# jvmncs/safe-grid-agents

Hardware: AMD Instinct MI355X
Metric: env-steps/sec at 1M concurrent BoatRace envs (higher is better)
Workload: dtype int8

## Files before the change

### safe-grid-agents_amd/csrc/sgk_api.hip

```cpp
#include <hip/hip_runtime.h>

#include <algorithm>
#include <cmath>
#include <cstdio>
#include <cstdlib>
#include <cstring>
#include <memory>
#include <utility>

#include "sgk_host_core.h"
#include "sgk_kernels.h"

using sgk::host::fail;
using sgk::host::GraphCache;
using sgk::host::hip_fail;
using sgk::host::KeepError;

namespace {

__global__ void set_counter_kernel(uint64_t *ctr, uint64_t v) { *ctr = v; }
__global__ void add_counter_kernel(uint64_t *ctr, uint64_t v) { *ctr += v; }

}

// ... 175 lines not shown
  if (n_envs <= 0 || n_envs > ((int64_t)1 << 31) - 512) return fail(SGK_ERR_INVALID, "n_envs out of range");
  const bool host_visible = (layout & SGK_MEM_HOST_VISIBLE) != 0;
  layout &= ~SGK_MEM_HOST_VISIBLE;
  if (layout != SGK_LAYOUT_PITCHED && layout != SGK_LAYOUT_COMPACT) return fail(SGK_ERR_INVALID, "unknown layout");
  if (host_visible && n_envs > 65536) return fail(SGK_ERR_INVALID, "SGK_MEM_HOST_VISIBLE is for small batches (<= 65536 envs)");
  int n_dev = 0;
  hipError_t e = hipGetDeviceCount(&n_dev);
  if (e != hipSuccess || n_dev <= 0)
    return fail(SGK_ERR_NODEVICE, "libsgk has no CPU fallback and found no HIP device%s%s", e != hipSuccess ? ": " : "",
                e != hipSuccess ? hipGetErrorString(e) : "");
  if (device < 0 || device >= n_dev) return fail(SGK_ERR_INVALID, "device ordinal out of range");
  sgk_env *h = sgk::host::host_new<sgk_env>();
  sgk::Shard &s = h->sh;
  if (sgk_build_rules(env_id, &s.rules_host) != 0) {
    delete h;
    return fail(SGK_ERR_INVALID, "unknown env_id");
  }
  s.env_id = env_id;
  s.device = device;
  s.n = n_envs;
  s.seed = seed;
  s.env_base = env_index_base;
  s.n_cells = s.rules_host.n_cells;
  s.n_states = s.rules_host.n_states;
  const int pitched = ((s.n_cells + 15) / 16) * 16;
  s.layout = layout;
  s.pitch = (s.layout == SGK_LAYOUT_COMPACT) ? s.n_cells : pitched;
  const char *ng = getenv("SGK_NO_GRAPH");
  h->use_graph = !(ng && ng[0] == '1');

#define SGK_TRY(call)                                   \
  do {                                                  \
    hipError_t e__ = (call);                            \
    if (e__ != hipSuccess) {                            \
      int rc__ = hip_fail(e__, #call);                  \
      const KeepError keep__;                           \
      sgk_destroy(h);                                   \
      keep__.restore();                                 \
      return rc__;                                      \
    }                                                   \
  } while (0)

  SGK_TRY(hipSetDevice(device));
  hipDeviceProp_t prop;
  SGK_TRY(hipGetDeviceProperties(&prop, device));
  s.n_cus = prop.multiProcessorCount > 0 ? prop.multiProcessorCount : 256;
  s.max_grid = s.n_cus * 6;
  if (const char *mg = getenv("SGK_MAX_GRID")) {
    int v = atoi(mg);
    if (v >= 64) s.max_grid = v;
  }
  s.stream_grid = s.n_cus * 16;
  if (const char *nt = getenv("SGK_RING_NT")) s.ring_nt_mode = nt[0] == '0' ? 0 : (nt[0] == '1' ? 1 : -1);
  if (const char *sg = getenv("SGK_STREAM_GRID")) {
    int v = atoi(sg);
    if (v >= 64) s.stream_grid = v;
  }
  s.rollout_grid = s.n_cus * 12;
  SGK_TRY(pooled_stream(device, &h->own_stream));
  h->stream = h->own_stream;
  const int64_t n_pad = ((s.n + 255) / 256) * 256;
  const int64_t n_wg = n_pad / 256;
  SGK_TRY(hipMalloc((void **)&s.rules_dev, sgk::SGK_RULES_DEV_BYTES));
  h->host_visible = host_visible;
  if (host_visible) {
    SGK_TRY(hipHostMalloc((void **)&s.state, sizeof(uint64_t) * n_pad, hipHostMallocMapped));
    SGK_TRY(hipHostMalloc((void **)&s.rec, sizeof(uint32_t) * n_pad, hipHostMallocMapped));
    SGK_TRY(hipHostMalloc((void **)&s.boards, (size_t)s.pitch * n_pad, hipHostMallocMapped));
    SGK_TRY(hipHostMalloc((void **)&h->hv_actions, (size_t)n_pad, hipHostMallocMapped));
    const char *srv = getenv("SGK_STEP_SERVER");
    if (n_envs <= 64 && !(srv && srv[0] == '0')) {
      SGK_TRY(hipHostMalloc((void **)&h->srv.mb, sizeof(sgk::SgkMailbox), hipHostMallocMapped));
      memset((void *)h->srv.mb, 0, sizeof(sgk::SgkMailbox));
    }
  } else {
    SGK_TRY(hipMalloc(&s.state, sizeof(uint64_t) * n_pad));
    SGK_TRY(hipMalloc(&s.rec, sizeof(uint32_t) * n_pad));
    SGK_TRY(hipMalloc(&s.boards, (size_t)s.pitch * n_pad));
  }
  if (host_visible) {
    SGK_TRY(hipHostMalloc((void **)&s.last_return, sizeof(int32_t) * n_pad, hipHostMallocMapped));
    SGK_TRY(hipHostMalloc((void **)&s.last_perf, sizeof(int32_t) * n_pad, hipHostMallocMapped));
  } else {
    SGK_TRY(hipMalloc(&s.last_return, sizeof(int32_t) * n_pad));
    SGK_TRY(hipMalloc(&s.last_perf, sizeof(int32_t) * n_pad));
  }
  SGK_TRY(hipMalloc(&s.n_episodes, sizeof(int32_t) * n_pad));
  SGK_TRY(hipMalloc(&s.n_resets, sizeof(int32_t) * n_pad));
  if (env_id == SGK_FRIEND_FOE) SGK_TRY(hipMalloc(&s.aux, sizeof(double) * SGK_AUX_DOUBLES * n_pad));
  SGK_TRY(hipMalloc(&s.metrics, sizeof(int64_t) * SGK_METRICS_LEN));
  SGK_TRY(hipMalloc(&s.metric_slab, sizeof(int64_t) * SGK_METRICS_LEN * SGK_METRIC_SLOTS));
  SGK_TRY(hipMalloc(&s.wg_count, sizeof(int32_t) * n_wg));
  SGK_TRY(hipMalloc(&s.wg_offset, sizeof(int64_t) * n_wg));
  SGK_TRY(hipMalloc(&s.finished_total, sizeof(int64_t)));
  SGK_TRY(hipMalloc(&h->t_dev, sizeof(uint64_t)));
  SGK_TRY(hipHostMalloc((void **)&h->metrics_pinned, sizeof(long long) * SGK_METRICS_LEN, hipHostMallocMapped));
  {
    static_assert(sgk::SGK_RULES_DEV_BYTES <= 8192, "staged on the stack");
    uint8_t image[sgk::SGK_RULES_DEV_BYTES];
    memset(image, 0, sizeof(image));
    memcpy(image, &s.rules_host, sizeof(SgkRules));
    for (int e = 0; e < 64; ++e) memcpy(image + sgk::SGK_RULES_IMAGE_BYTES + e * s.n_cells, s.rules_host.templ, (size_t)s.n_cells);
    SGK_TRY(hipMemcpyAsync(s.rules_dev, image, sizeof(image), hipMemcpyHostToDevice, h->stream));
    SGK_TRY(sgk::host::wait_stream(h->stream));
  }
  SGK_TRY(hipMemsetAsync(s.rec, 0, sizeof(uint32_t) * n_pad, h->stream));
// ... 1235 lines not shown
```

### safe-grid-agents_amd/csrc/sgk_device.h

```cpp
#pragma once
#include <hip/hip_runtime.h>
#include <limits.h>
#include <stdint.h>

#include "sgk_kernels.h"
#include "sgk_transition.h"


namespace sgk {

constexpr int WG = 256;

__device__ __forceinline__ int wave_index() { return __builtin_amdgcn_readfirstlane((int)(threadIdx.x >> 6)); }

template <class P>
__device__ __forceinline__ int keep_in_sgpr(P p) {
  asm volatile("" ::"s"(p));
  return 0;
}
template <class... P>
__device__ __forceinline__ void keep_in_sgprs(P... p) {
  (void)(keep_in_sgpr(p) + ...);
}

// ... 307 lines not shown
      }
      return;
    } else if (was != now) {
      const uint8_t *t = ALT ? backdrop_of(R, info_backdrop(now)) : R.templ;
      const int pos = was & 0xffu;
      row[pos] = t[pos];
      if (HasSprite2<ENV>::value) {
        const int box = (was >> 8) & 0xffu;
        if (box < NC) row[box] = t[box];
      }
    }
    __builtin_amdgcn_wave_barrier();
    if (was != now) poke(R, now);
  }

  template <int AUX = BOARD_STORE_AUX>
  __device__ __forceinline__ void flush(int8_t *dst) const {
    const int lane = threadIdx.x & 63;
    __builtin_amdgcn_wave_barrier();
    const __amdgpu_buffer_rsrc_t rsrc = __builtin_amdgcn_make_buffer_rsrc((void *)dst, 0, BYTES, 0x00020000);
    uint4 v[ITS];
#pragma unroll
    for (int it = 0; it < ITS; ++it) {
      const int j = lane + 64 * it;
      const int jr = (ITS * 64 == CHUNKS || j < CHUNKS) ? j : CHUNKS - 1;
      v[it] = *reinterpret_cast<const uint4 *>(tile + 16 * jr);
    }
#pragma unroll
    for (int it = 0; it < ITS; ++it) {
      sgk_u32x4 v4 = {v[it].x, v[it].y, v[it].z, v[it].w};
      __builtin_amdgcn_raw_buffer_store_b128(v4, rsrc, (lane + 64 * it) * 16, 0, AUX);
    }
    __builtin_amdgcn_wave_barrier();
  }

  __device__ __forceinline__ void flush_prefix(int8_t *dst, int n_bytes) const {
    const int lane = threadIdx.x & 63;
    __builtin_amdgcn_wave_barrier();
#pragma unroll
    for (int it = 0; it < ITS; ++it) {
      const int j = lane + 64 * it;
      if (j * 16 < n_bytes) reinterpret_cast<uint4 *>(dst)[j] = *reinterpret_cast<const uint4 *>(tile + 16 * j);
    }
    __builtin_amdgcn_wave_barrier();
  }

  __device__ __forceinline__ void write(const CompactLds<NC> &C, const SgkRules &R, uint32_t info, int8_t *dst) const {
    draw_all(C, R, info);
    flush(dst);
  }
};

template <int ENV, int NC>
__device__ __noinline__ void write_row_bytes(const SgkRules &R, int8_t *__restrict__ row, const EnvState &s) {
  const uint8_t *backdrop = HasAltBackdrop<ENV>::value ? backdrop_of(R, alt_backdrop<ENV>(R, s)) : R.templ;
  const bool shows_mask = HasMask<ENV>::value && !alt_backdrop<ENV>(R, s);
  const uint32_t mask = (uint32_t)s.box | ((uint32_t)s.ext << 8);
  for (int c = 0; c < NC; ++c) {
    uint8_t v = backdrop[c];
    if (HasSprite2<ENV>::value && c == s.box) v = (uint8_t)sprite2_value<ENV>(R, s);
    if (shows_mask && R.tomato_index[c] != 255 && ((mask >> R.tomato_index[c]) & 1u)) v = (uint8_t)R.value_box;
    if (c == s.pos) v = R.agent_value[c];
    row[c] = (int8_t)v;
  }
}

template <int ENV>
struct Geom;
template <>
struct Geom<SGK_BOAT_RACE> { static constexpr int NC = 25, PITCH = 32; };
template <>
struct Geom<SGK_ISLAND_NAVIGATION> { static constexpr int NC = 48, PITCH = 48; };
template <>
struct Geom<SGK_SIDE_EFFECTS_SOKOBAN> { static constexpr int NC = 36, PITCH = 48; };
template <>
struct Geom<SGK_DISTRIBUTIONAL_SHIFT> { static constexpr int NC = 63, PITCH = 64; };
template <>
struct Geom<SGK_WHISKY_GOLD> { static constexpr int NC = 48, PITCH = 48; };
template <>
struct Geom<SGK_ABSENT_SUPERVISOR> { static constexpr int NC = 48, PITCH = 48; };
template <>
struct Geom<SGK_SAFE_INTERRUPTIBILITY> { static constexpr int NC = 56, PITCH = 64; };
template <>
struct Geom<SGK_CONVEYOR_BELT> { static constexpr int NC = 49, PITCH = 64; };
template <>
struct Geom<SGK_TOMATO_WATERING> { static constexpr int NC = 63, PITCH = 64; };
template <>
struct Geom<SGK_FRIEND_FOE> { static constexpr int NC = 30, PITCH = 32; };

__device__ __forceinline__ double uniform53(uint32_t a, uint32_t b) {
  return (double)((((uint64_t)(a >> 5)) << 26) + (uint64_t)(b >> 6)) / 9007199254740992.0;
}

struct StepArgs {
  const SgkRules *rules;
  uint64_t *state;
  const uint8_t *actions;
  uint32_t *rec;
  int8_t *boards;
  int32_t *last_return, *last_perf, *n_episodes, *n_resets;
  double *aux;
  long long *metrics;
  int64_t n;
  uint64_t seed, env_base, t;
  const uint64_t *t_ptr;
  uint32_t flags;
};

template <int ENV>
__device__ __forceinline__ double *aux_of(double *aux, int64_t env) {
  return HasAux<ENV>::value ? aux + env * SGK_AUX_DOUBLES : nullptr;
}

template <int ENV>
__device__ __forceinline__ void step_one(const SgkRules &R, const StepArgs &a, int64_t env, bool valid, int action,
                                         EnvState &s, uint32_t &rec, EpisodeAcc &acc) {
  bool finished = false;
  int r_obs = 0, r_hid = 0;
  if (valid && !s.over) {
    int term;
    action = env_actual_action<ENV>(R, s, a.seed, a.env_base + (uint64_t)env, action);
    transition<ENV>(R, s, action, r_obs, r_hid, term, aux_of<ENV>(a.aux, env));
    s.frame += 1;
    s.ret += r_obs;
    s.hid += r_hid;
    finished = term || s.frame >= R.max_iterations;
  }
  int done = (valid && (s.over || finished)) ? 1 : 0;
  rec = pack_rec(r_obs, r_hid, done, action);
  acc_add(acc, finished, s.ret, s.hid);
  if (finished) {
    a.last_return[env] = s.ret;
    a.last_perf[env] = s.hid;
    bump_episode_count(a.n_episodes, env);
    if (a.flags & SGK_F_AUTO_RESET) {
      const int epi = s.epi + 1;
      bump_reset_count<ENV>(a.n_resets, env);
      s = initial_state(R);
      s.epi = epi;
      begin_episode<ENV>(R, s, a.seed, a.env_base + (uint64_t)env, aux_of<ENV>(a.aux, env));
    } else {
// ... 83 lines not shown
```

### safe-grid-agents_amd/csrc/sgk_kernels.h

```cpp
#pragma once
#include <hip/hip_runtime.h>
#include <stdint.h>

#include "../../include/sgk.h"
#include "sgk_mailbox.h"
#include "sgk_rules.h"

#define SGK_METRIC_SLOTS 2048

namespace sgk {

constexpr int SGK_RULES_IMAGE_BYTES = 2048;
constexpr int SGK_RULES_DEV_BYTES = SGK_RULES_IMAGE_BYTES + 64 * SGK_CELLS;

struct Shard {
  int env_id = 0, layout = 0, device = 0;
  int n_cells = 0, pitch = 0, n_states = 0;
  int n_cus = 256, max_grid = 2048, stream_grid = 2048, rollout_grid = 2048;
  int ring_nt_mode = -1;
  int64_t n = 0;
  uint64_t seed = 0, env_base = 0, lockstep_t = 0;
  SgkRules rules_host;
  SgkRules *rules_dev = nullptr;
  uint64_t *state = nullptr;
  uint32_t *rec = nullptr;
  int8_t *boards = nullptr;
  int32_t *last_return = nullptr;
  int32_t *last_perf = nullptr;
  int32_t *n_episodes = nullptr;
  int32_t *n_resets = nullptr;
  double *aux = nullptr;
  int64_t *metrics = nullptr;
  int64_t *metric_slab = nullptr;
  int32_t *wg_count = nullptr;
  int64_t *wg_offset = nullptr;
  int64_t *finished_total = nullptr;
};

struct TabqShard {
  double *table = nullptr;
  uint64_t *tags = nullptr;
  double *row_cache = nullptr;
  uint32_t *keys = nullptr;
  int32_t hash_cap = 0;
  int32_t *hash_overflow = nullptr;
  int32_t n_states = 0;
  double lr = 0, discount = 0, eps0 = 0;
  int64_t anneal = 0;
  int64_t t_agent = 0;
  const long long *t_ptr = nullptr;
};

hipError_t launch_step(const Shard &sh, const uint8_t *actions, uint32_t flags, hipStream_t st);
hipError_t launch_env_server(const Shard &sh, const uint8_t *actions, SgkMailbox *mb, uint32_t last, hipStream_t st);
hipError_t launch_rollout_random(const Shard &sh, int32_t n_steps, uint32_t flags, hipStream_t st);
hipError_t launch_rollout_stream(const Shard &sh, int32_t n_steps, uint32_t flags, int8_t *boards_ring, uint32_t *recs_ring,
                                 int32_t ring, int32_t slice0, hipStream_t st);
hipError_t launch_reset(const Shard &sh, const uint8_t *mask, int mode, hipStream_t st);
hipError_t launch_ring_probe(const Shard &sh, int8_t *boards_ring, uint32_t *recs_ring, int32_t ring, uint32_t flags, hipStream_t st);
hipError_t launch_metrics_init(const Shard &sh, hipStream_t st);
hipError_t launch_aux_init(const Shard &sh, hipStream_t st);
hipError_t launch_metrics_reduce(const Shard &sh, hipStream_t st, long long *out_host = nullptr);
hipError_t launch_obs_f32(const Shard &sh, float *dst, hipStream_t st);
struct PolicyWeights {
  const float *w1t, *b1, *w2, *b2, *w3t, *b3;
  int n_hidden;
};
hipError_t launch_policy_act(const Shard &sh, int mode, const PolicyWeights &w, uint8_t *actions, float *scores, double eps,
                             uint64_t draw, const double *eps_dev, const uint64_t *draw_dev, hipStream_t st);
hipError_t launch_policy_rollout(const Shard &sh, int mode, const PolicyWeights &w, double eps, uint64_t draw0, int32_t n_steps,
                                 uint32_t flags, int8_t *states_out, uint8_t *actions_out, uint32_t *recs_out, hipStream_t st);
// ... 108 lines not shown
```

### safe-grid-agents_amd/csrc/sgk_step.hip

```cpp
#include <type_traits>

#include "sgk_device.h"
#include "sgk_step_store.h"

namespace sgk {

constexpr int STREAM_MIN_WAVES = 4;
#define SGK_TILE_DECLARE(ENV, NC, ON)                                                 \
  __shared__ __attribute__((aligned(16))) uint8_t tile_images[WG / 64][64 * (NC)];    \
  WaveTileLds<ENV, NC> W;                                                             \
  W.bind(tile_images[wave_index()]);                                                  \
  if (ON) stage_rotations(C, R)
#define SGK_TILE_WRITE(INFO, DST) W.write(C, R, (INFO), (DST))

__global__ __launch_bounds__(1024) void metrics_reduce_kernel(const long long *__restrict__ slab, long long *__restrict__ out,
                                                              long long *__restrict__ out_host) {
  __shared__ long long part[1024];
  const int col = threadIdx.x & 15, lane_slot = threadIdx.x >> 4;
  const bool is_max = col >= SGK_M_MAX_RETURN && col <= SGK_M_MAX_MARGIN_POS;
  long long acc = is_max ? LLONG_MIN : 0;
  for (int sl = lane_slot; sl < SGK_METRIC_SLOTS; sl += 256) {
    long long v0 = slab[(size_t)sl * SGK_METRICS_LEN + col];
    long long v1 = slab[(size_t)(sl + 64) * SGK_METRICS_LEN + col];
    long long v2 = slab[(size_t)(sl + 128) * SGK_METRICS_LEN + col];
    long long v3 = slab[(size_t)(sl + 192) * SGK_METRICS_LEN + col];
    acc = is_max ? max(max(acc, v0), max(max(v1, v2), v3)) : acc + ((v0 + v1) + (v2 + v3));
  }
  part[threadIdx.x] = acc;
  __syncthreads();
  for (int half = 32; half >= 1; half >>= 1) {
    if (lane_slot < half) {
      long long o = part[(lane_slot + half) * 16 + col];
      part[threadIdx.x] = is_max ? max(part[threadIdx.x], o) : part[threadIdx.x] + o;
    }
    __syncthreads();
  }
  if (threadIdx.x < 16) {
    out[threadIdx.x] = part[threadIdx.x];
    if (out_host) out_host[threadIdx.x] = part[threadIdx.x];
  }
}

__global__ __launch_bounds__(WG) void metrics_init_kernel(long long *__restrict__ slab) {
  for (int i = blockIdx.x * WG + threadIdx.x; i < SGK_METRIC_SLOTS * SGK_METRICS_LEN; i += gridDim.x * WG) {
    int col = i & 15;
    slab[i] = (col >= SGK_M_MAX_RETURN && col <= SGK_M_MAX_MARGIN_POS) ? LLONG_MIN : 0;
  }
}

constexpr int64_t STEP_SMALL_MAX_ENVS = 65536;

template <int ENV, int LAYOUT, bool RANDOM, bool SMALL, bool STORE = false>
__global__ __launch_bounds__(SMALL ? 64 : WG) void step_kernel(StepArgs a, StepStore st) {
  constexpr int WGT = SMALL ? 64 : WG;
  constexpr int NC = Geom<ENV>::NC;
  constexpr bool COMPACT = (LAYOUT == SGK_LAYOUT_COMPACT);
  __shared__ WaveRulesImage rules_images[WGT / 64];
  __shared__ __attribute__((aligned(16))) uint8_t tile_images[COMPACT ? WGT / 64 : 1][COMPACT ? 64 * NC : 16];
  __shared__ int episode_words[WGT / 64][16];
// ... 140 lines not shown
      if (valid) {
        const int epi = s.epi + 1;
        bump_reset_count<ENV>(a.n_resets, env);
        s = initial_state(R);
        s.epi = epi;
        begin_episode<ENV>(R, s, a.seed, a.env_base + (uint64_t)env, aux_of<ENV>(a.aux, env));
        a.state[env] = pack_state(s);
      }
    } else {
      StepArgs b = a;
      b.flags = flags;
      uint32_t rec;
      step_one<ENV>(R, b, env, valid, action, s, rec, acc);
      if (valid) {
        a.state[env] = pack_state(s);
        a.rec[env] = rec;
      }
    }
    if (!(flags & SGK_F_NO_BOARDS)) {
      if (COMPACT) {
        W.draw_all(C, R, sprite_info<ENV>(R, s));
        W.flush_prefix(a.boards, (int)a.n * NC);
      } else if (valid) {
        write_board_pitched<ENV, Geom<ENV>::PITCH>(R, a.boards, env, s);
      }
    }
    __builtin_amdgcn_fence(__ATOMIC_RELEASE, "");
    asm volatile("s_waitcnt vmcnt(0)" ::: "memory");
    if (lane == 0) __hip_atomic_store(&mb->done, req, __ATOMIC_RELAXED, __HIP_MEMORY_SCOPE_SYSTEM);
    last = req;
  }
  acc_flush(acc, a.metrics);
  __builtin_amdgcn_fence(__ATOMIC_RELEASE, "");
  asm volatile("s_waitcnt vmcnt(0)" ::: "memory");
  if (lane == 0) __hip_atomic_store(&mb->exited, last + 1u, __ATOMIC_RELAXED, __HIP_MEMORY_SCOPE_SYSTEM);
}

hipError_t launch_env_server(const Shard &sh, const uint8_t *actions, SgkMailbox *mb, uint32_t last, hipStream_t st) {
  (void)hipGetLastError();
  StepArgs a = make_step_args(sh, actions, 0);
  SGK_DISPATCH_ENV_LAYOUT(sh.env_id, sh.layout, env_server_kernel<E, L><<<dim3(1), dim3(64), 0, st>>>(a, mb, last));
  return hipGetLastError();
}

struct StreamOut {
  int8_t *boards;
  uint32_t *recs;
  int32_t ring, slice0;
  int32_t tiles_ok;
  int32_t tile_major;
  int32_t ring_nt;
};

template <int ENV, int LAYOUT, bool STREAM>
__global__ __launch_bounds__(WG, STREAM ? STREAM_MIN_WAVES : 1) void rollout_random_kernel(StepArgs a, int32_t n_steps, StreamOut o) {
  constexpr int NC = Geom<ENV>::NC;
  constexpr bool COMPACT = (LAYOUT == SGK_LAYOUT_COMPACT);
  __shared__ SgkRules R;
  __shared__ CompactLds<NC> C;
  uint64_t first_word = 0;
  {
    const int64_t env0 = ((int64_t)blockIdx.x * (WG / 64) + (threadIdx.x >> 6)) * 64 + (threadIdx.x & 63);
    if (STREAM && env0 < a.n) first_word = a.state[env0];
  }
  stage_rules(R, a.rules);
  SGK_TILE_DECLARE(ENV, NC, (COMPACT || STREAM));
  const int lane = threadIdx.x & 63, wave = STREAM ? wave_index() : (int)(threadIdx.x >> 6);
  const bool boards_on = !(a.flags & SGK_F_NO_BOARDS);
  const int64_t n_wt = (a.n + 63) / 64;
  EpisodeAcc acc;
  acc_init(acc);
  for (int64_t wt = (int64_t)blockIdx.x * (WG / 64) + wave; wt < n_wt; wt += (int64_t)gridDim.x * (WG / 64)) {
    const int64_t env = wt * 64 + lane;
    const bool valid = env < a.n;
    EnvState s = initial_state(R);
    if (valid) s = unpack_state((STREAM && wt < (int64_t)gridDim.x * (WG / 64)) ? first_word : a.state[env]);
    load_episode_index<ENV>(s, a.n_resets, env, valid);
    const uint64_t ge = a.env_base + (uint64_t)env;
    AuxRegs ax;
    ax.init();
    if (HasAux<ENV>::value && valid) ax.load(a.aux + env * SGK_AUX_DOUBLES);
    uint32_t x[4] = {0, 0, 0, 0};
    uint32_t rec = 0;
    uint32_t w = 0;
    int last_obs = 0, last_hid = 0, last_done = 0, last_action = 0;
    const bool auto_reset = (a.flags & SGK_F_AUTO_RESET) != 0;
    const bool whole_tile = wt * 64 + 64 <= a.n;
    int32_t slice = o.slice0;
    uint32_t drawn = sprite_info<ENV>(R, s);
    if (STREAM && boards_on) W.draw_all(C, R, drawn);
    if (STREAM) {
    const bool tm = o.boards && o.tile_major;
    const bool tiles = o.boards ? (tm || (o.tiles_ok && whole_tile)) : COMPACT;
    const bool flush_nt = o.boards && o.ring_nt;
    uint32_t *recs_p = !o.recs ? a.rec + env
                               : (o.tile_major ? o.recs + (wt * (int64_t)o.ring + slice) * 64 + lane : o.recs + (int64_t)slice * a.n + env);
    const int64_t rec_stride = !o.recs ? 0 : (o.tile_major ? 64 : a.n);
    int8_t *dense = !o.boards ? a.boards
                              : (tm ? o.boards + ((wt * (int64_t)o.ring + slice) - wt) * 64 * NC : o.boards + (int64_t)slice * a.n * NC);
    const int64_t brd_stride = !o.boards ? 0 : (tm ? (int64_t)64 * NC : a.n * (int64_t)NC);
    const int64_t rec_wrap = rec_stride * (o.ring - 1), brd_wrap = brd_stride * (o.ring - 1);
    uint32_t left = 0;
#pragma nounroll
    for (int32_t k = 0; k < n_steps; ++k) {
      if (left == 0) {
        const uint64_t t = a.t + (uint64_t)k;
        const uint32_t tl = (uint32_t)t;
        if (k == 0 || (tl & 63u) == 0)
// ... 95 lines not shown
              s.over = 1;
            }
          }
        } else {
          last_obs = 0;
          last_hid = 0;
          last_done = valid ? 1 : 0;
        }
      };
      const bool lean = auto_reset && whole_tile && (__ballot(s.over != 0) == 0ull);
      uint64_t t = a.t;
      int32_t k = 0;
      bool have_block = false;
#pragma nounroll
      while (k < n_steps) {
        const uint32_t tl = (uint32_t)t;
        if (!have_block || (tl & 63u) == 0u) {
          philox4x32_10((uint32_t)ge, (uint32_t)(ge >> 32), (uint32_t)(t >> 6), 0u, (uint32_t)a.seed, (uint32_t)(a.seed >> 32), x);
          have_block = true;
        }
        const uint32_t j = (tl >> 4) & 3u;
        w = (j == 0 ? x[0] : (j == 1 ? x[1] : (j == 2 ? x[2] : x[3]))) >> (2 * (tl & 15u));
        const int32_t m = min((int32_t)(16u - (tl & 15u)), n_steps - k);
        if (lean) {
#pragma nounroll
          for (int32_t i = 0; i < m; ++i) {
            one_step((int)(w & 3u), std::false_type{});
            w >>= 2;
          }
        } else {
#pragma nounroll
          for (int32_t i = 0; i < m; ++i) {
            one_step((int)(w & 3u), std::true_type{});
            w >>= 2;
          }
        }
        k += m;
        t += (uint64_t)m;
      }
    }
    rec = pack_rec(last_obs, last_hid, last_done, last_action);
    if (valid) {
      a.state[env] = pack_state(s);
      if (!STREAM || o.recs) a.rec[env] = rec;
      if (HasEnvDraws<ENV>::value) a.n_resets[env] = s.epi;
      if (HasAux<ENV>::value && ax.dirty) ax.store(a.aux + env * SGK_AUX_DOUBLES);
    }
    if (!STREAM && boards_on) {
      if (COMPACT) SGK_TILE_WRITE(sprite_info<ENV>(R, s), a.boards + wt * 64 * NC);
      else if (valid) write_board_pitched<ENV, Geom<ENV>::PITCH>(R, a.boards, env, s);
    }
  }
  acc_flush(acc, a.metrics);
}

template <int ENV, int LAYOUT, bool STORE = false>
__global__ __launch_bounds__(WG) void reset_kernel(const SgkRules *rules, uint64_t *state, int8_t *boards,
                                                   const uint8_t *mask, int mode_flags, int64_t n, uint64_t seed, uint64_t env_base,
                                                   int32_t *__restrict__ n_resets, const double *__restrict__ aux, StepStore st) {
  reset_body<ENV, LAYOUT, STORE>(rules, state, boards, mask, mode_flags, n, seed, env_base, n_resets, aux, st, (int)blockIdx.x, (int)gridDim.x);
}

__global__ __launch_bounds__(WG) void obs_f32_kernel(const int8_t *__restrict__ boards, float *__restrict__ dst, int64_t n,
                                                     int nc, int pitch) {
  const int q_per_env = (nc + 3) / 4;
  const int64_t total = n * q_per_env;
  for (int64_t i = (int64_t)blockIdx.x * blockDim.x + threadIdx.x; i < total; i += (int64_t)gridDim.x * blockDim.x) {
    int64_t env = i / q_per_env;
    int q = (int)(i - env * q_per_env);
    const int8_t *src = boards + env * pitch + q * 4;
    float *out = dst + env * nc + q * 4;
    if (q * 4 + 4 <= nc && ((nc & 3) == 0) && ((pitch & 3) == 0)) {
      uint32_t w = *reinterpret_cast<const uint32_t *>(src);
      float4 f = make_float4((float)(int8_t)(w & 0xff), (float)(int8_t)((w >> 8) & 0xff),
                             (float)(int8_t)((w >> 16) & 0xff), (float)(int8_t)(w >> 24));
      *reinterpret_cast<float4 *>(out) = f;
    } else {
      for (int k = 0; k < 4 && q * 4 + k < nc; ++k) out[k] = (float)src[k];
    }
  }
}

__global__ __launch_bounds__(WG) void render_rgb_kernel(const SgkRules *__restrict__ rules, const int8_t *__restrict__ boards,
                                                        uint8_t *__restrict__ dst, int64_t n, int nc, int pitch) {
  __shared__ uint8_t pal[8][4];
  if (threadIdx.x < 32) (&pal[0][0])[threadIdx.x] = (&rules->palette[0][0])[threadIdx.x];
  __syncthreads();
  const bool hwc = rules->render_hwc != 0;
  const int64_t total = n * nc;
  for (int64_t i = (int64_t)blockIdx.x * blockDim.x + threadIdx.x; i < total; i += (int64_t)gridDim.x * blockDim.x) {
    int64_t env = i / nc;
    int c = (int)(i - env * nc);
    int v = boards[env * pitch + c] & 7;
    uint8_t *o = dst + env * 3 * nc + (hwc ? 3 * c : c);
    const int plane = hwc ? 1 : nc;
    o[0] = pal[v][0];
    o[plane] = pal[v][1];
    o[2 * plane] = pal[v][2];
  }
}

__global__ __launch_bounds__(WG) void dense_boards_kernel(const int8_t *__restrict__ boards, int8_t *__restrict__ dst,
                                                          int64_t n, int nc, int pitch) {
  const int64_t total = n * nc;
  for (int64_t i = (int64_t)blockIdx.x * blockDim.x + threadIdx.x; i < total; i += (int64_t)gridDim.x * blockDim.x) {
    int64_t env = i / nc;
// ... 81 lines not shown
}

hipError_t launch_step(const Shard &sh, const uint8_t *actions, uint32_t flags, hipStream_t st) {
  (void)hipGetLastError();
  StepArgs a = make_step_args(sh, actions, flags);
  const bool small = sh.n <= STEP_SMALL_MAX_ENVS;
  const dim3 grid(small ? (unsigned)((sh.n + 63) / 64) : (unsigned)grid_for((sh.n + WG - 1) / WG, sh.max_grid)), block(small ? 64 : WG);
  if (actions) {
    if (small) SGK_DISPATCH_ENV_LAYOUT(sh.env_id, sh.layout, step_kernel<E, L, false, true><<<grid, block, 0, st>>>(a, StepStore{}));
    else SGK_DISPATCH_ENV_LAYOUT(sh.env_id, sh.layout, step_kernel<E, L, false, false><<<grid, block, 0, st>>>(a, StepStore{}));
  } else {
    if (small) SGK_DISPATCH_ENV_LAYOUT(sh.env_id, sh.layout, step_kernel<E, L, true, true><<<grid, block, 0, st>>>(a, StepStore{}));
    else SGK_DISPATCH_ENV_LAYOUT(sh.env_id, sh.layout, step_kernel<E, L, true, false><<<grid, block, 0, st>>>(a, StepStore{}));
  }
  return hipGetLastError();
}


hipError_t launch_step_store(const Shard &sh, const uint8_t *actions, uint32_t flags, int cheat, int64_t slice, const long long *slice_dev,
                             int32_t ring, int8_t *successors, uint8_t *r_actions, int8_t *r_rewards, uint8_t *r_terminals, hipStream_t st) {
  (void)hipGetLastError();
  StepArgs a = make_step_args(sh, actions, flags);
  const StepStore so = make_store(sh, successors, r_actions, r_rewards, r_terminals, slice, slice_dev, ring, cheat);
  const bool small = sh.n <= STEP_SMALL_MAX_ENVS;
  const dim3 grid(small ? (unsigned)((sh.n + 63) / 64) : (unsigned)grid_for((sh.n + WG - 1) / WG, sh.max_grid)), block(small ? 64 : WG);
  if (small) SGK_DISPATCH_ENV_LAYOUT(sh.env_id, sh.layout, step_kernel<E, L, false, true, true><<<grid, block, 0, st>>>(a, so));
  else SGK_DISPATCH_ENV_LAYOUT(sh.env_id, sh.layout, step_kernel<E, L, false, false, true><<<grid, block, 0, st>>>(a, so));
  return hipGetLastError();
}

hipError_t launch_rollout_random(const Shard &sh, int32_t n_steps, uint32_t flags, hipStream_t st) {
  (void)hipGetLastError();
  StepArgs a = make_step_args(sh, nullptr, flags);
  int grid = grid_for((sh.n + WG - 1) / WG, sh.rollout_grid);
  StreamOut o{nullptr, nullptr, 1, 0, 0, 0, 0};
  SGK_DISPATCH_ENV_LAYOUT(sh.env_id, sh.layout,
                          rollout_random_kernel<E, L, false><<<dim3(grid), dim3(WG), 0, st>>>(a, n_steps, o));
  return hipGetLastError();
}

static int32_t ring_stores_nt(const Shard &sh, int64_t ring_bytes, int32_t ring_slices) {
  if (sh.ring_nt_mode >= 0) return sh.ring_nt_mode;
  return ring_slices >= 48 && ring_bytes > (256ll << 20);
}

hipError_t launch_rollout_stream(const Shard &sh, int32_t n_steps, uint32_t flags, int8_t *boards_ring, uint32_t *recs_ring,
                                 int32_t ring, int32_t slice0, hipStream_t st) {
  (void)hipGetLastError();
  StepArgs a = make_step_args(sh, nullptr, flags);
  int grid = grid_for((sh.n + WG - 1) / WG, sh.stream_grid);
  StreamOut o{boards_ring, recs_ring, ring < 1 ? 1 : ring, slice0, (int32_t)(((sh.n * sh.n_cells) % 16) == 0 && ((uintptr_t)boards_ring % 16) == 0),
              (int32_t)((flags & SGK_F_RING_TILE_MAJOR) != 0),
              ring_stores_nt(sh, (int64_t)(ring < 1 ? 1 : ring) * sh.n * (sh.n_cells + 4), ring)};
  SGK_DISPATCH_ENV_LAYOUT(sh.env_id, sh.layout,
                          rollout_random_kernel<E, L, true><<<dim3(grid), dim3(WG), 0, st>>>(a, n_steps, o));
  hipError_t e = hipGetLastError();
  if (e != hipSuccess) return e;
  const bool in_kernel = sh.layout == SGK_LAYOUT_COMPACT && (o.tile_major || (o.tiles_ok && sh.n % 64 == 0));
  if (boards_ring && !(flags & SGK_F_NO_BOARDS) && !in_kernel) return launch_reset(sh, nullptr, 2, st);
  return hipSuccess;
}

template <int NC>
__global__ __launch_bounds__(WG) void ring_probe_kernel(int8_t *boards, uint32_t *recs, int64_t n, int32_t ring, int32_t tile_major,
                                                       int32_t nt) {
  constexpr int BYTES = 64 * NC, CHUNKS = 4 * NC, ITS = (CHUNKS + 63) / 64;
  const int lane = threadIdx.x & 63, wave = wave_index();
  const int64_t n_wt = n / 64;
  const sgk_u32x4 zero = {0u, 0u, 0u, 0u};
  for (int64_t wt = (int64_t)blockIdx.x * (WG / 64) + wave; wt < n_wt; wt += (int64_t)gridDim.x * (WG / 64)) {
    for (int32_t s = 0; s < ring; ++s) {
      if (boards) {
        int8_t *dst = tile_major ? boards + (wt * (int64_t)ring + s) * BYTES : boards + ((int64_t)s * n + wt * 64) * NC;
        const __amdgpu_buffer_rsrc_t rsrc = __builtin_amdgcn_make_buffer_rsrc((void *)dst, 0, BYTES, 0x00020000);
#pragma unroll
        for (int it = 0; it < ITS; ++it) {
          if (nt) __builtin_amdgcn_raw_buffer_store_b128(zero, rsrc, (lane + 64 * it) * 16, 0, RING_STORE_AUX);
          else __builtin_amdgcn_raw_buffer_store_b128(zero, rsrc, (lane + 64 * it) * 16, 0, BOARD_STORE_AUX);
        }
      }
      if (recs) {
        uint32_t *r = tile_major ? recs + (wt * (int64_t)ring + s) * 64 + lane : recs + (int64_t)s * n + wt * 64 + lane;
        *r = 0u;
      }
    }
  }
}

hipError_t launch_ring_probe(const Shard &sh, int8_t *boards_ring, uint32_t *recs_ring, int32_t ring, uint32_t flags, hipStream_t st) {
  (void)hipGetLastError();
  int grid = grid_for((sh.n + WG - 1) / WG, sh.stream_grid);
  const int32_t tm = (flags & SGK_F_RING_TILE_MAJOR) != 0;
  const int32_t nt = ring_stores_nt(sh, (int64_t)ring * sh.n * (sh.n_cells + 4), ring);
  SGK_DISPATCH_ENV(sh.env_id, (ring_probe_kernel<Geom<E>::NC><<<dim3(grid), dim3(WG), 0, st>>>(boards_ring, recs_ring, sh.n, ring, tm, nt)));
  return hipGetLastError();
}

hipError_t launch_reset(const Shard &sh, const uint8_t *mask, int mode, hipStream_t st) {
  (void)hipGetLastError();
  int grid = grid_for((sh.n + WG - 1) / WG, sh.max_grid);
  SGK_DISPATCH_ENV_LAYOUT(sh.env_id, sh.layout,
                          reset_kernel<E, L><<<dim3(grid), dim3(WG), 0, st>>>(sh.rules_dev, sh.state,
                                              sh.boards, mask, mode, sh.n, sh.seed, sh.env_base, sh.n_resets, sh.aux, StepStore{}));
  return hipGetLastError();
}

hipError_t launch_reset_done_store(const Shard &sh, uint32_t flags, int64_t slice, const long long *slice_dev, int32_t ring, int8_t *states,
                                   hipStream_t st) {
// ... 70 lines not shown
```

Before: 176.6 billion.

## Process two 64-env tiles per wave in BoatRace streamed rollout

Adds a streamed rollout variant for BoatRace in which each wave handles two adjacent 64-env tiles (128 envs). The two tiles' steps are interleaved for extra instruction-level parallelism, and both boards go out in one contiguous buffer-store flush of 128*NC bytes. The variant uses a lower launch-bounds occupancy target and half the grid, and is on by default unless SGK_STREAM_TPW=1. In exchange it doubles per-wave LDS and register state, which may lower occupancy.

New measurement: 178.2 billion, median of 6. About the same (+0.9%).

```diff
diff --git a/safe-grid-agents_amd/csrc/sgk_api.hip b/safe-grid-agents_amd/csrc/sgk_api.hip
--- a/safe-grid-agents_amd/csrc/sgk_api.hip
+++ b/safe-grid-agents_amd/csrc/sgk_api.hip
@@ -251,6 +251,7 @@
   }
   s.stream_grid = s.n_cus * 16;
   if (const char *nt = getenv("SGK_RING_NT")) s.ring_nt_mode = nt[0] == '0' ? 0 : (nt[0] == '1' ? 1 : -1);
+  if (const char *tp = getenv("SGK_STREAM_TPW")) s.stream_tpw = (tp[0] == '1' && tp[1] == 0) ? 1 : 0;
   if (const char *sg = getenv("SGK_STREAM_GRID")) {
     int v = atoi(sg);
     if (v >= 64) s.stream_grid = v;
diff --git a/safe-grid-agents_amd/csrc/sgk_device.h b/safe-grid-agents_amd/csrc/sgk_device.h
--- a/safe-grid-agents_amd/csrc/sgk_device.h
+++ b/safe-grid-agents_amd/csrc/sgk_device.h
@@ -383,6 +383,39 @@
 };
 
 template <int ENV, int NC>
+struct WavePairLds {
+  static constexpr int BYTES = 128 * NC, CHUNKS = 8 * NC, ITS = (CHUNKS + 63) / 64;
+  WaveTileLds<ENV, NC> half[2];
+  uint8_t *image;
+
+  __device__ __forceinline__ void bind(uint8_t *wave_image) {
+    image = wave_image;
+    half[0].bind(wave_image);
+    half[1].bind(wave_image + 64 * NC);
+  }
+
+  template <int AUX = BOARD_STORE_AUX>
+  __device__ __forceinline__ void flush(int8_t *dst) const {
+    const int lane = threadIdx.x & 63;
+    __builtin_amdgcn_wave_barrier();
+    const __amdgpu_buffer_rsrc_t rsrc = __builtin_amdgcn_make_buffer_rsrc((void *)dst, 0, BYTES, 0x00020000);
+    uint4 v[ITS];
+#pragma unroll
+    for (int it = 0; it < ITS; ++it) {
+      const int j = lane + 64 * it;
+      const int jr = (ITS * 64 == CHUNKS || j < CHUNKS) ? j : CHUNKS - 1;
+      v[it] = *reinterpret_cast<const uint4 *>(image + 16 * jr);
+    }
+#pragma unroll
+    for (int it = 0; it < ITS; ++it) {
+      sgk_u32x4 v4 = {v[it].x, v[it].y, v[it].z, v[it].w};
+      __builtin_amdgcn_raw_buffer_store_b128(v4, rsrc, (lane + 64 * it) * 16, 0, AUX);
+    }
+    __builtin_amdgcn_wave_barrier();
+  }
+};
+
+template <int ENV, int NC>
 __device__ __noinline__ void write_row_bytes(const SgkRules &R, int8_t *__restrict__ row, const EnvState &s) {
   const uint8_t *backdrop = HasAltBackdrop<ENV>::value ? backdrop_of(R, alt_backdrop<ENV>(R, s)) : R.templ;
   const bool shows_mask = HasMask<ENV>::value && !alt_backdrop<ENV>(R, s);
@@ -418,6 +451,11 @@
 struct Geom<SGK_TOMATO_WATERING> { static constexpr int NC = 63, PITCH = 64; };
 template <>
 struct Geom<SGK_FRIEND_FOE> { static constexpr int NC = 30, PITCH = 32; };
+
+template <int ENV>
+struct StreamTilesPerWave { static constexpr int value = 1; };
+template <>
+struct StreamTilesPerWave<SGK_BOAT_RACE> { static constexpr int value = 2; };
 
 __device__ __forceinline__ double uniform53(uint32_t a, uint32_t b) {
   return (double)((((uint64_t)(a >> 5)) << 26) + (uint64_t)(b >> 6)) / 9007199254740992.0;
diff --git a/safe-grid-agents_amd/csrc/sgk_kernels.h b/safe-grid-agents_amd/csrc/sgk_kernels.h
--- a/safe-grid-agents_amd/csrc/sgk_kernels.h
+++ b/safe-grid-agents_amd/csrc/sgk_kernels.h
@@ -17,6 +17,7 @@
   int env_id = 0, layout = 0, device = 0;
   int n_cells = 0, pitch = 0, n_states = 0;
   int n_cus = 256, max_grid = 2048, stream_grid = 2048, rollout_grid = 2048;
+  int stream_tpw = 0;
   int ring_nt_mode = -1;
   int64_t n = 0;
   uint64_t seed = 0, env_base = 0, lockstep_t = 0;
diff --git a/safe-grid-agents_amd/csrc/sgk_step.hip b/safe-grid-agents_amd/csrc/sgk_step.hip
--- a/safe-grid-agents_amd/csrc/sgk_step.hip
+++ b/safe-grid-agents_amd/csrc/sgk_step.hip
@@ -5,6 +5,10 @@
 
 namespace sgk {
 
+#ifndef SGK_PAIRS_MIN_WAVES
+#define SGK_PAIRS_MIN_WAVES 3
+#endif
+constexpr int PAIRS_MIN_WAVES = SGK_PAIRS_MIN_WAVES;
 constexpr int STREAM_MIN_WAVES = 4;
 #define SGK_TILE_DECLARE(ENV, NC, ON)                                                 \
   __shared__ __attribute__((aligned(16))) uint8_t tile_images[WG / 64][64 * (NC)];    \
@@ -251,8 +255,170 @@
   int32_t ring_nt;
 };
 
-template <int ENV, int LAYOUT, bool STREAM>
-__global__ __launch_bounds__(WG, STREAM ? STREAM_MIN_WAVES : 1) void rollout_random_kernel(StepArgs a, int32_t n_steps, StreamOut o) {
+template <int ENV, int LAYOUT>
+__device__ __forceinline__ void rollout_pairs_body(const StepArgs &a, int32_t n_steps, const StreamOut &o) {
+  constexpr int NC = Geom<ENV>::NC;
+  constexpr bool COMPACT = (LAYOUT == SGK_LAYOUT_COMPACT);
+  __shared__ SgkRules R;
+  __shared__ CompactLds<NC> C;
+  __shared__ __attribute__((aligned(16))) uint8_t pair_images[WG / 64][128 * NC];
+  const int lane = threadIdx.x & 63, wave = wave_index();
+  const int64_t pair0 = (int64_t)blockIdx.x * (WG / 64) + wave, pstride = (int64_t)gridDim.x * (WG / 64);
+  uint64_t first_word[2] = {0, 0};
+#pragma unroll
+  for (int h = 0; h < 2; ++h) {
+    const int64_t env0 = pair0 * 128 + h * 64 + lane;
+    if (env0 < a.n) first_word[h] = a.state[env0];
+  }
+  stage_rules(R, a.rules);
+  WavePairLds<ENV, NC> W;
+  W.bind(pair_images[wave]);
+  stage_rotations(C, R);
+  const bool boards_on = !(a.flags & SGK_F_NO_BOARDS);
+  const bool auto_reset = (a.flags & SGK_F_AUTO_RESET) != 0;
+  const bool flush_nt = o.ring_nt != 0;
+  const int64_t n_pairs = (a.n + 127) / 128;
+  EpisodeAcc acc;
+  acc_init(acc);
+  for (int64_t p = pair0; p < n_pairs; p += pstride) {
+    const int64_t env_lo = p * 128 + lane;
+    const bool pair_whole = p * 128 + 128 <= a.n;
+    bool valid[2], tile_whole[2];
+    EnvState s[2];
+    AuxRegs ax[2];
+    uint32_t x[2][4] = {{0, 0, 0, 0}, {0, 0, 0, 0}}, w[2] = {0, 0}, drawn[2];
+    int last_obs[2] = {0, 0}, last_hid[2] = {0, 0}, last_done[2] = {0, 0}, last_action[2] = {0, 0};
+#pragma unroll
+    for (int h = 0; h < 2; ++h) {
+      const int64_t env = env_lo + 64 * h;
+      valid[h] = env < a.n;
+      tile_whole[h] = p * 128 + 64 * h + 64 <= a.n;
+      s[h] = initial_state(R);
+      if (valid[h]) s[h] = unpack_state(p == pair0 ? first_word[h] : a.state[env]);
+      load_episode_index<ENV>(s[h], a.n_resets, env, valid[h]);
+      ax[h].init();
+      if (HasAux<ENV>::value && valid[h]) ax[h].load(a.aux + env * SGK_AUX_DOUBLES);
+      drawn[h] = sprite_info<ENV>(R, s[h]);
+      if (boards_on) W.half[h].draw_all(C, R, drawn[h]);
+    }
+    const uint64_t ge_lo = a.env_base + (uint64_t)env_lo;
+    int32_t slice = o.slice0;
+    uint32_t *recs_p = !o.recs ? a.rec + env_lo : o.recs + (int64_t)slice * a.n + env_lo;
+    const int64_t rec_stride = !o.recs ? 0 : a.n;
+    int8_t *dense = o.boards + (int64_t)slice * a.n * NC;
+    const int64_t brd_stride = a.n * (int64_t)NC;
+    const int64_t rec_wrap = rec_stride * (o.ring - 1), brd_wrap = brd_stride * (o.ring - 1);
+    uint32_t left = 0;
+#pragma nounroll
+    for (int32_t k = 0; k < n_steps; ++k) {
+      const bool new_word = left == 0;
+      const uint64_t t = a.t + (uint64_t)k;
+      const uint32_t tl = (uint32_t)t;
+      if (new_word) left = 16 - (tl & 15u);
+      --left;
+#pragma unroll
+      for (int h = 0; h < 2; ++h) {
+        const uint64_t ge = ge_lo + 64u * h;
+        if (new_word) {
+          if (k == 0 || (tl & 63u) == 0)
+            philox4x32_10((uint32_t)ge, (uint32_t)(ge >> 32), (uint32_t)(t >> 6), 0u, (uint32_t)a.seed, (uint32_t)(a.seed >> 32), x[h]);
+          const uint32_t j = (tl >> 4) & 3u;
+          w[h] = (j == 0 ? x[h][0] : (j == 1 ? x[h][1] : (j == 2 ? x[h][2] : x[h][3]))) >> (2 * (tl & 15u));
+        }
+        int action = (int)(w[h] & 3u);
+        w[h] >>= 2;
+        const bool live = valid[h] && !s[h].over;
+        if (live) action = env_actual_action<ENV>(R, s[h], a.seed, ge, action);
+        last_action[h] = action;
+        last_obs[h] = 0;
+        last_hid[h] = 0;
+        last_done[h] = valid[h] ? 1 : 0;
+        if (live) {
+          int r_obs, r_hid, term;
+          if (HasAux<ENV>::value) transition_with<ENV>(R, s[h], action, r_obs, r_hid, term, ax[h]);
+          else transition<ENV>(R, s[h], action, r_obs, r_hid, term);
+          s[h].frame += 1;
+          s[h].ret += r_obs;
+          s[h].hid += r_hid;
+          last_obs[h] = r_obs;
+          last_hid[h] = r_hid;
+          last_done[h] = 0;
+          if (term || s[h].frame >= R.max_iterations) {
+            last_done[h] = 1;
+            acc_add(acc, true, s[h].ret, s[h].hid);
+            int64_t env_here = env_lo + 64 * h;
+            asm volatile("" : "+v"(env_here));
+            a.last_return[env_here] = s[h].ret;
+            a.last_perf[env_here] = s[h].hid;
+            bump_episode_count(a.n_episodes, env_here);
+            if (auto_reset) {
+              const int epi = s[h].epi + 1;
+              s[h] = initial_state(R);
+              s[h].epi = epi;
+              if (HasAux<ENV>::value) begin_episode_with<ENV>(R, s[h], a.seed, ge, ax[h]);
+              else begin_episode<ENV>(R, s[h], a.seed, ge);
+            } else {
+              s[h].over = 1;
+            }
+          }
+        }
+        if (valid[h]) recs_p[64 * h] = pack_rec(last_obs[h], last_hid[h], last_done[h], last_action[h]);
+        if (boards_on) {
+          const uint32_t now = sprite_info<ENV>(R, s[h]);
+          W.half[h].update(R, drawn[h], now);
+          drawn[h] = now;
+        }
+      }
+      if (boards_on) {
+        if (pair_whole) {
+          if (flush_nt) W.template flush<RING_STORE_AUX>(dense + p * 128 * NC);
+          else W.flush(dense + p * 128 * NC);
+        } else {
+#pragma unroll
+          for (int h = 0; h < 2; ++h) {
+            if (tile_whole[h]) {
+              if (flush_nt) W.half[h].template flush<RING_STORE_AUX>(dense + (p * 2 + h) * 64 * NC);
+              else W.half[h].flush(dense + (p * 2 + h) * 64 * NC);
+            } else if (valid[h]) {
+              write_row_bytes<ENV, NC>(R, dense + (env_lo + 64 * h) * NC, s[h]);
+            }
+          }
+        }
+      }
+      if (++slice == o.ring) {
+        slice = 0;
+        recs_p -= rec_wrap;
+        dense -= brd_wrap;
+      } else {
+        recs_p += rec_stride;
+        dense += brd_stride;
+      }
+    }
+    if (boards_on && COMPACT && n_steps > 0) {
+      if (pair_whole) W.flush(a.boards + p * 128 * NC);
+      else if (tile_whole[0]) W.half[0].flush(a.boards + p * 128 * NC);
+    }
+#pragma unroll
+    for (int h = 0; h < 2; ++h) {
+      const int64_t env = env_lo + 64 * h;
+      if (valid[h]) {
+        a.state[env] = pack_state(s[h]);
+        if (o.recs) a.rec[env] = pack_rec(last_obs[h], last_hid[h], last_done[h], last_action[h]);
+        if (HasEnvDraws<ENV>::value) a.n_resets[env] = s[h].epi;
+        if (HasAux<ENV>::value && ax[h].dirty) ax[h].store(a.aux + env * SGK_AUX_DOUBLES);
+      }
+    }
+  }
+  acc_flush(acc, a.metrics);
+}
+
+template <int ENV, int LAYOUT, bool STREAM, int TPW = 1>
+__global__ __launch_bounds__(WG, STREAM ? (TPW == 2 ? PAIRS_MIN_WAVES : STREAM_MIN_WAVES) : 1) void rollout_random_kernel(StepArgs a, int32_t n_steps, StreamOut o) {
+  static_assert(TPW == 1 || (TPW == 2 && STREAM), "two tiles per wave: the streamed form only");
+  if constexpr (TPW == 2) {
+    rollout_pairs_body<ENV, LAYOUT>(a, n_steps, o);
+    return;
+  } else {
   constexpr int NC = Geom<ENV>::NC;
   constexpr bool COMPACT = (LAYOUT == SGK_LAYOUT_COMPACT);
   __shared__ SgkRules R;
@@ -454,6 +620,7 @@
     }
   }
   acc_flush(acc, a.metrics);
+  }
 }
 
 template <int ENV, int LAYOUT, bool STORE = false>
@@ -641,8 +808,18 @@
   StreamOut o{boards_ring, recs_ring, ring < 1 ? 1 : ring, slice0, (int32_t)(((sh.n * sh.n_cells) % 16) == 0 && ((uintptr_t)boards_ring % 16) == 0),
               (int32_t)((flags & SGK_F_RING_TILE_MAJOR) != 0),
               ring_stores_nt(sh, (int64_t)(ring < 1 ? 1 : ring) * sh.n * (sh.n_cells + 4), ring)};
-  SGK_DISPATCH_ENV_LAYOUT(sh.env_id, sh.layout,
-                          rollout_random_kernel<E, L, true><<<dim3(grid), dim3(WG), 0, st>>>(a, n_steps, o));
+  const bool pairs = sh.stream_tpw != 1 && boards_ring && o.tiles_ok && !o.tile_major;
+  const int pair_grid = grid_for((sh.n + 2 * WG - 1) / (2 * WG), sh.stream_grid);
+  SGK_DISPATCH_ENV_LAYOUT(sh.env_id, sh.layout, {
+    if constexpr (StreamTilesPerWave<E>::value == 2) {
+      if (pairs) rollout_random_kernel<E, L, true, 2><<<dim3(pair_grid), dim3(WG), 0, st>>>(a, n_steps, o);
+      else rollout_random_kernel<E, L, true><<<dim3(grid), dim3(WG), 0, st>>>(a, n_steps, o);
+    } else {
+      rollout_random_kernel<E, L, true><<<dim3(grid), dim3(WG), 0, st>>>(a, n_steps, o);
+    }
+  });
+  (void)pairs;
+  (void)pair_grid;
   hipError_t e = hipGetLastError();
   if (e != hipSuccess) return e;
   const bool in_kernel = sh.layout == SGK_LAYOUT_COMPACT && (o.tile_major || (o.tiles_ok && sh.n % 64 == 0));
```
